# xl-tang3/RCOT

Measured on AMD Instinct MI355X. Metric: 128x128 patches/sec (gen+critic step), higher is better.
Workload: dtype fp32 (exact fp32 MFMA everywhere); 1 GPU; BASELINE configs[1]: Restormer T_net(decoder=True)+F_net(128), denoise_50, RMSprop, paired, B=8/GPU 128x128; global_batch=8, patch=128, parallelism=dp1, gemm_prec=fp32

## Files before the change

### rcot_amd/csrc/pointwise.hip

```cpp
#include <cstdlib>
#include "common.h"
#include "../../include/rcot_hip.h"

using namespace rcot;

namespace {

constexpr int LN_TX = 16, LN_TY = 16, LN_PIX = LN_TX * 4;

__device__ __forceinline__ float4 f4_add(float4 a, float4 b) { return make_float4(a.x + b.x, a.y + b.y, a.z + b.z, a.w + b.w); }

template <int TX>
__device__ __forceinline__ float4 reduce_rows(float4 v, float4* red, int tx, int ty) {
    constexpr int TY = 256 / TX;
    __syncthreads();
    red[ty * TX + tx] = v;
    __syncthreads();
    float4 t = red[tx];
#pragma unroll
    for (int i = 1; i < TY; ++i) t = f4_add(t, red[i * TX + tx]);
    return t;
}

__global__ __launch_bounds__(256) void ln_stats_kernel(const float* __restrict__ x, float* __restrict__ mu,
                                                       float* __restrict__ rs, int C, int N) {
    __shared__ float4 red[256];
    const int tx = threadIdx.x & (LN_TX - 1), ty = threadIdx.x >> 4;
    const int n = blockIdx.x * LN_PIX + tx * 4;
    const int b = blockIdx.y;
    const bool ok = n < N;
    const float* p = x + (long)b * C * N + (ok ? n : 0);
    const float4 sh = ok ? *reinterpret_cast<const float4*>(p) : make_float4(0, 0, 0, 0);
    float4 s = make_float4(0, 0, 0, 0), ss = make_float4(0, 0, 0, 0);
    if (ok) {
#pragma unroll 4
        for (int c = ty; c < C; c += LN_TY) {
            const float4 v = *reinterpret_cast<const float4*>(p + (long)c * N);
            const float dx_ = v.x - sh.x, dy_ = v.y - sh.y, dz_ = v.z - sh.z, dw_ = v.w - sh.w;
            s.x += dx_; s.y += dy_; s.z += dz_; s.w += dw_;
            ss.x += dx_ * dx_; ss.y += dy_ * dy_; ss.z += dz_ * dz_; ss.w += dw_ * dw_;
        }
    }
    s = reduce_rows<LN_TX>(s, red, tx, ty);
    ss = reduce_rows<LN_TX>(ss, red, tx, ty);
    if (ty == 0 && ok) {
        const float inv = 1.0f / (float)C;
        float4 m, r;
#define RCOT_LN_FIN(q)                                              \
    {                                                               \
        const float e = s.q * inv;                                  \
        const float var = fmaxf(ss.q * inv - e * e, 0.f);           \
        m.q = sh.q + e;                                             \
        r.q = 1.0f / sqrtf(var + 1e-5f);                            \
    }
        RCOT_LN_FIN(x) RCOT_LN_FIN(y) RCOT_LN_FIN(z) RCOT_LN_FIN(w)
#undef RCOT_LN_FIN
        *reinterpret_cast<float4*>(mu + (long)b * N + n) = m;
        *reinterpret_cast<float4*>(rs + (long)b * N + n) = r;
    }
}

template <int NC, int TX>
__global__ __launch_bounds__(256) void ln_bwd_kernel(const float* __restrict__ g, const float* __restrict__ x,
                                                     const float* __restrict__ mu, const float* __restrict__ rs,
                                                     const float* __restrict__ w, const float* __restrict__ dres,
                                                     float* __restrict__ dx, float* __restrict__ part, int C, int N) {
    constexpr int TY = 256 / TX, PIX = TX * 4;
    __shared__ float4 red[256];
    __shared__ float sdw[512], sdb[512];
    const int tid = threadIdx.x;
    const int tx = tid % TX, ty = tid / TX;
    const int b = blockIdx.y;
    for (int c = tid; c < C; c += 256) { sdw[c] = 0.f; sdb[c] = 0.f; }
    __syncthreads();
    const int ntiles = (N + PIX - 1) / PIX;
    for (int tile = blockIdx.x; tile < ntiles; tile += gridDim.x) {
        const int n = tile * PIX + tx * 4;
        const bool ok = n < N;
        const long base = (long)b * C * N + (ok ? n : 0);
        const float4 m = ok ? *reinterpret_cast<const float4*>(mu + (long)b * N + n) : make_float4(0, 0, 0, 0);
        const float4 r = ok ? *reinterpret_cast<const float4*>(rs + (long)b * N + n) : make_float4(0, 0, 0, 0);
        float4 s1 = make_float4(0, 0, 0, 0), s2 = make_float4(0, 0, 0, 0);
        constexpr int NR = NC > 0 ? NC : 1;
        float4 gk[NR], xk[NR];
        const int niter = NC > 0 ? NC : (C - ty + TY - 1) / TY;
#pragma unroll
        for (int it = 0; it < NR; ++it) { gk[it] = make_float4(0, 0, 0, 0); xk[it] = gk[it]; }
        if (NC > 0 && ok) {
#pragma unroll
            for (int it = 0; it < NR; ++it) {
                const long i = base + (long)(ty + it * TY) * N;
                gk[it] = *reinterpret_cast<const float4*>(g + i);
                xk[it] = *reinterpret_cast<const float4*>(x + i);
            }
        }
        for (int it = 0; it < niter; ++it) {
            const int c = ty + it * TY;
            float4 gv = make_float4(0, 0, 0, 0), xh = gv;
            if (NC > 0) {
#pragma unroll
                for (int q = 0; q < NR; ++q)
                    if (q == it) { gv = gk[q]; xh = xk[q]; }
                xh = make_float4((xh.x - m.x) * r.x, (xh.y - m.y) * r.y, (xh.z - m.z) * r.z, (xh.w - m.w) * r.w);
#pragma unroll
                for (int q = 0; q < NR; ++q)
                    if (q == it) xk[q] = xh;
            } else if (ok) {
                gv = *reinterpret_cast<const float4*>(g + base + (long)c * N);
                const float4 xv = *reinterpret_cast<const float4*>(x + base + (long)c * N);
                xh = make_float4((xv.x - m.x) * r.x, (xv.y - m.y) * r.y, (xv.z - m.z) * r.z, (xv.w - m.w) * r.w);
            }
            const float wc = w[c];
            s1.x += gv.x * wc; s1.y += gv.y * wc; s1.z += gv.z * wc; s1.w += gv.w * wc;
            s2.x += gv.x * wc * xh.x; s2.y += gv.y * wc * xh.y; s2.z += gv.z * wc * xh.z; s2.w += gv.w * wc * xh.w;
            float a = gv.x * xh.x + gv.y * xh.y + gv.z * xh.z + gv.w * xh.w;
            float bb = gv.x + gv.y + gv.z + gv.w;
#pragma unroll
            for (int o = TX / 2; o > 0; o >>= 1) {
                a += __shfl_xor(a, o, 64);
                bb += __shfl_xor(bb, o, 64);
            }
            if (tx == 0) {
                sdw[c] += a;
                sdb[c] += bb;
            }
        }
        s1 = reduce_rows<TX>(s1, red, tx, ty);
        s2 = reduce_rows<TX>(s2, red, tx, ty);
        if (ok) {
            const float inv = 1.0f / (float)C;
            s1.x *= inv; s1.y *= inv; s1.z *= inv; s1.w *= inv;
            s2.x *= inv; s2.y *= inv; s2.z *= inv; s2.w *= inv;
#pragma unroll
            for (int it = 0; it < NR; ++it) {
                if (NC == 0) break;
                const int c = ty + it * TY;
                const long i = base + (long)c * N;
                const float wc = w[c];
                float4 v;
                v.x = r.x * (gk[it].x * wc - s1.x - xk[it].x * s2.x);
                v.y = r.y * (gk[it].y * wc - s1.y - xk[it].y * s2.y);
                v.z = r.z * (gk[it].z * wc - s1.z - xk[it].z * s2.z);
                v.w = r.w * (gk[it].w * wc - s1.w - xk[it].w * s2.w);
                if (dres) v = f4_add(v, *reinterpret_cast<const float4*>(dres + i));
                *reinterpret_cast<float4*>(dx + i) = v;
            }
            if (NC == 0)
                for (int c = ty; c < C; c += TY) {
                    const long i = base + (long)c * N;
                    const float4 gv = *reinterpret_cast<const float4*>(g + i);
                    const float4 xv = *reinterpret_cast<const float4*>(x + i);
                    const float wc = w[c];
                    float4 v;
                    v.x = r.x * (gv.x * wc - s1.x - (xv.x - m.x) * r.x * s2.x);
                    v.y = r.y * (gv.y * wc - s1.y - (xv.y - m.y) * r.y * s2.y);
                    v.z = r.z * (gv.z * wc - s1.z - (xv.z - m.z) * r.z * s2.z);
                    v.w = r.w * (gv.w * wc - s1.w - (xv.w - m.w) * r.w * s2.w);
                    if (dres) v = f4_add(v, *reinterpret_cast<const float4*>(dres + i));
                    *reinterpret_cast<float4*>(dx + i) = v;
                }
        }
    }
    __syncthreads();
    float* row = part + ((long)blockIdx.y * gridDim.x + blockIdx.x) * (2 * C);
    for (int c = tid; c < C; c += 256) {
        row[c] = sdw[c];
        row[C + c] = sdb[c];
    }
}

__global__ __launch_bounds__(1024) void ln_param_reduce_kernel(const float* __restrict__ part, int rows, int C,
                                                               float* __restrict__ dw, float* __restrict__ db) {
    __shared__ float red[32][33];
    const int cl = threadIdx.x & 31, rl = threadIdx.x >> 5;
    const int col = blockIdx.x * 32 + cl, C2 = 2 * C;
    float s0 = 0.f, s1 = 0.f;
    if (col < C2) {
        const float* p = part + col;
        int r = rl;
        for (; r + 32 < rows; r += 64) {
            s0 += p[(long)r * C2];
            s1 += p[(long)(r + 32) * C2];
        }
        if (r < rows) s0 += p[(long)r * C2];
    }
    red[rl][cl] = s0 + s1;
    __syncthreads();
    if (rl == 0 && col < C2) {
        float s = 0.f;
#pragma unroll
        for (int i = 0; i < 32; ++i) s += red[i][cl];
        if (col < C) dw[col] += s;
        else db[col - C] += s;
    }
}

struct SlabSets {
    const float* ws[4];
    float* dst[4];
    int S[4], M[4], N[4], ldws[4];
    int per[4];
    long ldd[4];
    int chunk0[5];
    int n;
};

__global__ __launch_bounds__(1024) void block_param_reduce_kernel(const float* __restrict__ part1, const float* __restrict__ part2,
                                                                  int rows, int C, float* __restrict__ gw1, float* __restrict__ gb1,
                                                                  float* __restrict__ gw2, float* __restrict__ gb2,
                                                                  const float* __restrict__ dWo_part, float* __restrict__ gWo,
                                                                  const float* __restrict__ dtemp_part, float* __restrict__ gtemp,
                                                                  int B, int heads, int nw, SlabSets ss) {
    __shared__ float red[32][33];
    const int nl = (2 * C + 31) / 32;
    const int blk = blockIdx.x;
    if (blk >= 2 * nl + nw) {
        const int cb = blk - 2 * nl - nw;
        int d = 0;
        while (d + 1 < ss.n && cb >= ss.chunk0[d + 1]) ++d;
        const int c = cb - ss.chunk0[d];
        const long mn = (long)ss.M[d] * ss.N[d];
        const long slab = (long)ss.M[d] * ss.ldws[d];
        if (ss.S[d] <= 8) {
            const unsigned Nn = (unsigned)ss.N[d], mnu = (unsigned)mn, S = (unsigned)ss.S[d];
            const unsigned ldw = (unsigned)ss.ldws[d];
            const float* wsb = ss.ws[d];
            float* dstb = ss.dst[d];
            float v[4][8], old[4];
            long doff[4];
            bool ok[4];
#pragma unroll
            for (int j = 0; j < 4; ++j) {
                const unsigned idx = (unsigned)c * 4096u + 1024u * j + threadIdx.x;
                ok[j] = idx < mnu;
                const unsigned ic = ok[j] ? idx : mnu - 1;
                const unsigned m = ic / Nn, n = ic - m * Nn;
                const float* w = wsb + (size_t)m * ldw + n;
                doff[j] = (long)m * ss.ldd[d] + n;
#pragma unroll
                for (unsigned u = 0; u < 8; ++u) {
                    const unsigned uc = u < S ? u : S - 1;
                    v[j][u] = w[(long)uc * slab];
                }
                old[j] = dstb[doff[j]];
            }
#pragma unroll
            for (int j = 0; j < 4; ++j) {
#pragma unroll
                for (unsigned u = 0; u < 8; ++u) v[j][u] = u < S ? v[j][u] : 0.f;
                const float sum = ((v[j][0] + v[j][1]) + (v[j][2] + v[j][3])) + ((v[j][4] + v[j][5]) + (v[j][6] + v[j][7]));
                if (ok[j]) dstb[doff[j]] = old[j] + sum;
            }
            return;
        }
        if (ss.per[d] == 256) {
            const int o = threadIdx.x & 255, q = threadIdx.x >> 8;
            const long idx = (long)c * 256 + o;
            float* part = &red[0][0];
            float a = 0.f;
            int m = 0, n = 0;
            if (idx < mn) {
                m = (int)(idx / ss.N[d]);
                n = (int)(idx - (long)m * ss.N[d]);
                const float* w = ss.ws[d] + (long)m * ss.ldws[d] + n;
                float acc8[8];
#pragma unroll
                for (int u = 0; u < 8; ++u) acc8[u] = 0.f;
                int s = q;
                for (; s + 28 < ss.S[d]; s += 32) {
#pragma unroll
                    for (int u = 0; u < 8; ++u) acc8[u] += w[(long)(s + 4 * u) * slab];
                }
                for (; s < ss.S[d]; s += 4) acc8[0] += w[(long)s * slab];
                a = ((acc8[0] + acc8[1]) + (acc8[2] + acc8[3])) + ((acc8[4] + acc8[5]) + (acc8[6] + acc8[7]));
            }
            part[q * 256 + o] = a;
            __syncthreads();
            if (q == 0 && idx < mn)
                ss.dst[d][(long)m * ss.ldd[d] + n] += (part[o] + part[256 + o]) + (part[512 + o] + part[768 + o]);
            return;
        }
        const int o = threadIdx.x & 255, q = threadIdx.x >> 8;
        const unsigned Nn = (unsigned)ss.N[d], mnu = (unsigned)mn, ldw = (unsigned)ss.ldws[d];
        const int S = ss.S[d];
        float a[4];
        long doff[4];
        bool ok[4];
        const float* w[4];
#pragma unroll
        for (int j = 0; j < 4; ++j) {
            const unsigned idx = (unsigned)c * 1024u + 256u * j + o;
            ok[j] = idx < mnu;
            const unsigned ic = ok[j] ? idx : mnu - 1;
            const unsigned m = ic / Nn, n = ic - m * Nn;
            w[j] = ss.ws[d] + (size_t)m * ldw + n;
            doff[j] = (long)m * ss.ldd[d] + n;
        }
        float acc8[4][8];
#pragma unroll
        for (int j = 0; j < 4; ++j)
#pragma unroll
            for (int u = 0; u < 8; ++u) acc8[j][u] = 0.f;
        int sl = q;
        for (; sl + 28 < S; sl += 32) {
#pragma unroll
            for (int j = 0; j < 4; ++j)
#pragma unroll
                for (int u = 0; u < 8; ++u) acc8[j][u] += w[j][(long)(sl + 4 * u) * slab];
        }
        for (; sl < S; sl += 4) {
#pragma unroll
            for (int j = 0; j < 4; ++j) acc8[j][0] += w[j][(long)sl * slab];
        }
#pragma unroll
        for (int j = 0; j < 4; ++j)
            a[j] = ((acc8[j][0] + acc8[j][1]) + (acc8[j][2] + acc8[j][3])) + ((acc8[j][4] + acc8[j][5]) + (acc8[j][6] + acc8[j][7]));
        __shared__ float part4[4][1024];
#pragma unroll
        for (int j = 0; j < 4; ++j) part4[q][256 * j + o] = a[j];
        __syncthreads();
        {
            const int t = threadIdx.x;
            const unsigned idx = (unsigned)c * 1024u + t;
            if (idx < mnu) {
                const unsigned m = idx / Nn, n = idx - m * Nn;
                ss.dst[d][(long)m * ss.ldd[d] + n] += (part4[0][t] + part4[1][t]) + (part4[2][t] + part4[3][t]);
            }
        }
        (void)doff; (void)ok;
        return;
    }
    if (blk < 2 * nl) {
        const float* part = blk < nl ? part1 : part2;
        float* dw = blk < nl ? gw1 : gw2;
        float* db = blk < nl ? gb1 : gb2;
        const int cb = blk < nl ? blk : blk - nl;
        const int cl = threadIdx.x & 31, rl = threadIdx.x >> 5;
        const int col = cb * 32 + cl, C2 = 2 * C;
        float a8[8];
#pragma unroll
        for (int u = 0; u < 8; ++u) a8[u] = 0.f;
        if (col < C2) {
            const float* p = part + col;
            int r = rl;
            for (; r + 224 < rows; r += 256) {
#pragma unroll
                for (int u = 0; u < 8; ++u) a8[u] += p[(long)(r + 32 * u) * C2];
            }
            for (; r < rows; r += 32) a8[0] += p[(long)r * C2];
        }
        red[rl][cl] = ((a8[0] + a8[1]) + (a8[2] + a8[3])) + ((a8[4] + a8[5]) + (a8[6] + a8[7]));
        __syncthreads();
        if (rl == 0 && col < C2) {
            float s = 0.f;
#pragma unroll
            for (int i = 0; i < 32; ++i) s += red[i][cl];
            if (col < C) dw[col] += s;
            else db[col - C] += s;
        }
        return;
    }
    const long n = (long)C * C;
    const long i = (long)(blk - 2 * nl) * 1024 + threadIdx.x;
    if (i < n) {
        float s = 0.f;
        int b = 0;
        for (; b + 8 <= B; b += 8) {
            float v[8];
#pragma unroll
            for (int u = 0; u < 8; ++u) v[u] = dWo_part[(long)(b + u) * n + i];
#pragma unroll
            for (int u = 0; u < 8; ++u) s += v[u];
        }
        for (; b < B; ++b) s += dWo_part[(long)b * n + i];
        gWo[i] += s;
    }
    if (blk == 2 * nl && threadIdx.x < heads) {
        float s = 0.f;
        for (int b = 0; b < B; ++b) s += dtemp_part[(long)b * heads + threadIdx.x];
        gtemp[threadIdx.x] += s;
    }
}

__global__ __launch_bounds__(256) void row_sumsq_kernel(const float* __restrict__ x, float* __restrict__ out, int R,
                                                        int N, long sXb) {
    __shared__ float red[4];
    const int r = blockIdx.x, b = blockIdx.y;
    const float* p = x + (long)b * sXb + (long)r * N;
    float s = 0.f;
#pragma unroll 4
    for (int n = threadIdx.x * 4; n < N; n += 1024) {
        const float4 v = *reinterpret_cast<const float4*>(p + n);
        s += v.x * v.x + v.y * v.y + v.z * v.z + v.w * v.w;
    }
    s = block_sum<256>(s, red);
    if (threadIdx.x == 0) out[(long)b * R + r] = s;
}

__global__ void lrelu_bwd_kernel(const float* __restrict__ dy, const float* __restrict__ a, float* __restrict__ dz,
                                 long n, float slope) {
    for (long i = (long)blockIdx.x * blockDim.x + threadIdx.x; i < n; i += (long)gridDim.x * blockDim.x)
        dz[i] = a[i] > 0.f ? dy[i] : dy[i] * slope;
}

__global__ __launch_bounds__(256) void bias_grad_kernel(const float* __restrict__ dz, float* __restrict__ db, int B,
                                                        int C, int P) {
    __shared__ float red[4];
    const int c = blockIdx.x;
    float s = 0.f;
    for (int b = 0; b < B; ++b) {
        const float* p = dz + ((long)b * C + c) * P;
#pragma unroll 8
        for (int i = threadIdx.x; i < P; i += 256) s += p[i];
    }
    s = block_sum<256>(s, red);
    if (threadIdx.x == 0) atomicAdd(&db[c], s);
}

__global__ void axpby2d_kernel(const float* x, long sx, const float* y, long sy, float* out, long so, long rows,
                               long cols, float a, float b) {
    const long n = rows * cols;
    for (long i = (long)blockIdx.x * blockDim.x + threadIdx.x; i < n; i += (long)gridDim.x * blockDim.x) {
        const long r = i / cols, c = i - r * cols;
        out[r * so + c] = a * x[r * sx + c] + (y ? b * y[r * sy + c] : 0.f);
    }
}

__global__ void fill_kernel(float* __restrict__ p, long n, float v) {
    const long head = min(n, (long)((4 - (((uintptr_t)p >> 2) & 3)) & 3));
    const long n4 = (n - head) >> 2;
    float4* q = reinterpret_cast<float4*>(p + head);
    const float4 v4 = make_float4(v, v, v, v);
    const long t0 = (long)blockIdx.x * blockDim.x + threadIdx.x, ts = (long)gridDim.x * blockDim.x;
    for (long i = t0; i < n4; i += ts) q[i] = v4;
    if (t0 < head) p[t0] = v;
    const long tail = head + 4 * n4;
    if (t0 < n - tail) p[tail + t0] = v;
}

__global__ void lerp_kernel(const float* __restrict__ t, const float* __restrict__ f, const float* __restrict__ alpha,
                            float* __restrict__ out, long per, long n) {
    for (long i = (long)blockIdx.x * blockDim.x + threadIdx.x; i < n; i += (long)gridDim.x * blockDim.x) {
        const float a = alpha[i / per];
        out[i] = a * t[i] + (1.f - a) * f[i];
    }
}

__global__ __launch_bounds__(256) void gp_norm_kernel(const float* __restrict__ g, float* __restrict__ norms, long per) {
    __shared__ float red[4];
    const float* p = g + (long)blockIdx.x * per;
    float s = 0.f;
    for (long i = threadIdx.x; i < per; i += 256) s += p[i] * p[i];
    s = block_sum<256>(s, red);
    if (threadIdx.x == 0) norms[blockIdx.x] = sqrtf(s);
}
__global__ void gp_scale_kernel(const float* __restrict__ g, const float* __restrict__ norms, float* __restrict__ u0,
                                float* __restrict__ gp_out, long per, int B, float inv_bg) {
    const long n = per * B;
    if (blockIdx.x == 0 && threadIdx.x == 0) {
        float s = 0.f;
        for (int b = 0; b < B; ++b) s += (norms[b] - 1.f) * (norms[b] - 1.f);
        *gp_out = 10.f * inv_bg * s;
    }
    for (long i = (long)blockIdx.x * blockDim.x + threadIdx.x; i < n; i += (long)gridDim.x * blockDim.x) {
        const float nm = norms[i / per];
        const float coef = nm > 0.f ? 20.f * inv_bg * (nm - 1.f) / nm : 0.f;
        u0[i] = coef * g[i];
    }
}

__global__ void pixel_shuffle_kernel(const float* __restrict__ in, float* __restrict__ out, long n, int H, int W, int mode) {
    for (long i = (long)blockIdx.x * blockDim.x + threadIdx.x; i < n; i += (long)gridDim.x * blockDim.x) {
        const int x = (int)(i % W);
        const long t = i / W;
        const int y = (int)(t % H);
        const long ch = t / H;
        long o;
        if (mode == 1) {
            const long oc = 4 * ch + 2 * (y & 1) + (x & 1);
            o = (oc * (H >> 1) + (y >> 1)) * (W >> 1) + (x >> 1);
        } else {
            const long oc = ch >> 2;
            const int ii = (int)((ch >> 1) & 1), jj = (int)(ch & 1);
            o = (oc * (2 * H) + (2 * y + ii)) * (2L * W) + (2 * x + jj);
        }
        out[o] = in[i];
    }
}

inline int ln_bwd_grid(int B, int N, bool* wide) {
    *wide = (long)cdiv(N, 64) * B >= 512;
    const int tiles = cdiv(N, *wide ? 64 : 16);
    int gx = 1024 / B;
    if (gx < 1) gx = 1;
    if (gx > tiles) gx = tiles;
    return gx;
}

}

extern "C" {

int rcot_ln_stats(const float* x, float* mu, float* rs, int B, int C, int N, void* stream) {
    if (!x || !mu || !rs || B <= 0 || C <= 0 || N <= 0) return RCOT_EINVAL;
    if ((N & 3) || (reinterpret_cast<uintptr_t>(x) & 15) || (reinterpret_cast<uintptr_t>(mu) & 15) ||
        (reinterpret_cast<uintptr_t>(rs) & 15))
        return RCOT_EINVAL;
    RCOT_LAUNCH(ln_stats_kernel, dim3(cdiv(N, LN_PIX), B), dim3(256), 0, (hipStream_t)stream, x, mu, rs, C, N);
    RCOT_LAUNCH_CHECK();
    return RCOT_OK;
}

int rcot_ln_bwd(const float* g, const float* x, const float* mu, const float* rs, const float* w, const float* dres,
                float* dx, float* dw, float* db, int B, int C, int N, void* ws, long ws_bytes, void* stream) {
    if (!g || !x || !mu || !rs || !w || !dx || !ws || B <= 0 || C <= 0 || C > 512 || N <= 0 || B > 65535) return RCOT_EINVAL;
    if ((dw == nullptr) != (db == nullptr)) return RCOT_EINVAL;
    if ((N & 3) || !al16(g) || !al16(x) || !al16(mu) || !al16(rs) || !al16(dx) || !al16(dres)) return RCOT_EINVAL;
    bool wide;
    const int gx = ln_bwd_grid(B, N, &wide);
    const long need = (long)gx * B * 2 * C * (long)sizeof(float);
    if (ws_bytes < need) return RCOT_EINVAL;
    float* part = static_cast<float*>(ws);
    const dim3 grid(gx, B);
    const int TY = wide ? 16 : 64;
    const int nc = (C % TY == 0 && (C / TY == 3 || C / TY == 6)) ? C / TY : 0;
#define RCOT_LNB(NC, TX) do { note_kernel("ln_bwd_kernel<%d, %d>", NC, TX); RCOT_LAUNCH((ln_bwd_kernel<NC, TX>), grid, dim3(256), 0, (hipStream_t)stream, g, x, mu, rs, w, dres, dx, part, C, N); } while (0)
    if (wide) {
        if (nc == 3) RCOT_LNB(3, 16);
        else if (nc == 6) RCOT_LNB(6, 16);
        else RCOT_LNB(0, 16);
    } else {
        if (nc == 3) RCOT_LNB(3, 4);
        else if (nc == 6) RCOT_LNB(6, 4);
        else RCOT_LNB(0, 4);
    }
#undef RCOT_LNB
    RCOT_LAUNCH_CHECK();
    if (dw) {
        RCOT_LAUNCH(ln_param_reduce_kernel, dim3(cdiv(2 * C, 32)), dim3(1024), 0, (hipStream_t)stream, part, gx * B, C, dw, db);
        RCOT_LAUNCH_CHECK();
    }
    return RCOT_OK;
}

int rcot_ln_bwd_rows(int B, int C, int N) {
    (void)C;
    if (B <= 0 || N <= 0) return 0;
    bool wide;
    return ln_bwd_grid(B, N, &wide) * B;
}

int rcot_block_param_reduce(const float* part1, const float* part2, int rows, int C, float* gw1, float* gb1, float* gw2,
                            float* gb2, const float* dWo_part, float* gWo, const float* dtemp_part, float* gtemp, int B,
                            int heads, const long long* slab_sets, int n_sets, void* stream) {
    if (!part1 || !part2 || !gw1 || !gb1 || !gw2 || !gb2 || !dWo_part || !gWo || !dtemp_part || !gtemp || rows <= 0 || C <= 0 ||
        B <= 0 || heads <= 0 || heads > 1024 || n_sets < 0 || n_sets > 4 || (n_sets && !slab_sets))
        return RCOT_EINVAL;
    const int nl = cdiv(2 * C, 32);
    const int nw = cdiv((long)C * C, 1024);
    SlabSets ss{};
    ss.n = n_sets;
    int chunks = 0;
    for (int d = 0; d < n_sets; ++d) {
        const long long* r = slab_sets + 7 * d;
        ss.ws[d] = reinterpret_cast<const float*>(r[0]);
        ss.S[d] = (int)r[1]; ss.M[d] = (int)r[2]; ss.N[d] = (int)r[3]; ss.ldws[d] = (int)r[4];
        ss.dst[d] = reinterpret_cast<float*>(r[5]);
        ss.ldd[d] = r[6];
        if (!ss.ws[d] || !ss.dst[d] || ss.S[d] <= 0 || ss.M[d] <= 0 || ss.N[d] <= 0 || ss.ldws[d] < ss.N[d]) return RCOT_EINVAL;
        ss.chunk0[d] = chunks;
        const long mn_ = (long)ss.M[d] * ss.N[d];
        ss.per[d] = ss.S[d] <= 8 ? 4096 : (mn_ >= 256 * 1024 ? 1024 : 256);
        chunks += cdiv(mn_, ss.per[d]);
    }
    ss.chunk0[n_sets] = chunks;
    RCOT_LAUNCH(block_param_reduce_kernel, dim3(2 * nl + nw + chunks), dim3(1024), 0, (hipStream_t)stream, part1, part2, rows,
                       C, gw1, gb1, gw2, gb2, dWo_part, gWo, dtemp_part, gtemp, B, heads, nw, ss);
    RCOT_LAUNCH_CHECK();
    return RCOT_OK;
}

int rcot_row_sumsq(const float* x, float* out, int B, int R, int N, long sXb, void* stream) {
    if (!x || !out || B <= 0 || R <= 0 || N <= 0 || (N & 3) || (sXb & 3) || !al16(x) || B > 65535) return RCOT_EINVAL;
    RCOT_LAUNCH(row_sumsq_kernel, dim3(R, B), dim3(256), 0, (hipStream_t)stream, x, out, R, N, sXb);
    RCOT_LAUNCH_CHECK();
    return RCOT_OK;
}

int rcot_lrelu_bwd(const float* dy, const float* a, float* dz, long n, float slope, void* stream) {
    if (!dy || !a || !dz || n <= 0) return RCOT_EINVAL;
    RCOT_LAUNCH(lrelu_bwd_kernel, dim3(grid_for(n)), dim3(256), 0, (hipStream_t)stream, dy, a, dz, n, slope);
    RCOT_LAUNCH_CHECK();
    return RCOT_OK;
}

int rcot_bias_grad(const float* dz, float* db, int B, int C, int P, void* stream) {
    if (!dz || !db || B <= 0 || C <= 0 || P <= 0) return RCOT_EINVAL;
    RCOT_LAUNCH(bias_grad_kernel, dim3(C), dim3(256), 0, (hipStream_t)stream, dz, db, B, C, P);
    RCOT_LAUNCH_CHECK();
    return RCOT_OK;
}

int rcot_axpby2d(const float* x, long sx, const float* y, long sy, float* out, long so, long rows, long cols, float a,
                 float b, void* stream) {
    if (!x || !out || rows <= 0 || cols <= 0) return RCOT_EINVAL;
    RCOT_LAUNCH(axpby2d_kernel, dim3(grid_for(rows * cols)), dim3(256), 0, (hipStream_t)stream, x, sx, y, sy, out,
                       so, rows, cols, a, b);
    RCOT_LAUNCH_CHECK();
    return RCOT_OK;
}

int rcot_fill(float* p, long n, float v, void* stream) {
    if (!p || n <= 0) return RCOT_EINVAL;
    RCOT_LAUNCH(fill_kernel, dim3(grid_for((n + 3) / 4)), dim3(256), 0, (hipStream_t)stream, p, n, v);
    RCOT_LAUNCH_CHECK();
    return RCOT_OK;
}

int rcot_lerp(const float* t, const float* f, const float* alpha, float* out, int B, long per, void* stream) {
    if (!t || !f || !alpha || !out || B <= 0 || per <= 0) return RCOT_EINVAL;
    RCOT_LAUNCH(lerp_kernel, dim3(grid_for(per * B)), dim3(256), 0, (hipStream_t)stream, t, f, alpha, out, per, per * B);
    RCOT_LAUNCH_CHECK();
    return RCOT_OK;
}

int rcot_gp_penalty(const float* g, float* norms, float* u0, float* gp_out, int B, long per, float inv_global_batch,
                    void* stream) {
    if (!g || !norms || !u0 || !gp_out || B <= 0 || per <= 0) return RCOT_EINVAL;
    RCOT_LAUNCH(gp_norm_kernel, dim3(B), dim3(256), 0, (hipStream_t)stream, g, norms, per);
    RCOT_LAUNCH_CHECK();
    RCOT_LAUNCH(gp_scale_kernel, dim3(grid_for(per * B)), dim3(256), 0, (hipStream_t)stream, g, norms, u0, gp_out,
                       per, B, inv_global_batch);
    RCOT_LAUNCH_CHECK();
    return RCOT_OK;
}

int rcot_pixel_shuffle(const float* in, float* out, long planes, int H, int W, int mode, void* stream) {
    if (!in || !out || planes <= 0 || H <= 0 || W <= 0 || (mode != 1 && mode != 2)) return RCOT_EINVAL;
    if (mode == 1 && ((H | W) & 1)) return RCOT_EINVAL;
    if (mode == 2 && (planes & 3)) return RCOT_EINVAL;
    const long n = planes * H * W;
    RCOT_LAUNCH(pixel_shuffle_kernel, dim3(grid_for(n)), dim3(256), 0, (hipStream_t)stream, in, out, n, H, W, mode);
    RCOT_LAUNCH_CHECK();
    return RCOT_OK;
}

}
```

Baseline: 107.2 patches/s.

## Restructure LayerNorm backward with register-held channels, wider blocks, and warp-shuffle reductions

Rewrites the LayerNorm backward kernel so the per-channel weight/bias gradient partials stay in registers across tiles instead of shared-memory accumulators. Block size now scales with C (256/512/1024 threads) so each thread holds a fixed 3 channels, with the residual gradient also loaded into registers. The column reductions for s1/s2 now use cross-lane shuffles plus a double-buffered small shared array with one barrier per tile. The kernel also uses 32-bit byte offsets and a waves-per-EU hint. This is meant to cut LDS traffic, barriers and reloads of g/x. In exchange there are more template variants and more register pressure.

```diff
diff --git a/rcot_amd/csrc/pointwise.hip b/rcot_amd/csrc/pointwise.hip
--- a/rcot_amd/csrc/pointwise.hip
+++ b/rcot_amd/csrc/pointwise.hip
@@ -60,112 +60,172 @@
     }
 }
 
-template <int NC, int TX>
-__global__ __launch_bounds__(256) void ln_bwd_kernel(const float* __restrict__ g, const float* __restrict__ x,
-                                                     const float* __restrict__ mu, const float* __restrict__ rs,
-                                                     const float* __restrict__ w, const float* __restrict__ dres,
-                                                     float* __restrict__ dx, float* __restrict__ part, int C, int N) {
-    constexpr int TY = 256 / TX, PIX = TX * 4;
-    __shared__ float4 red[256];
-    __shared__ float sdw[512], sdb[512];
+template <int LO, int HI>
+__device__ __forceinline__ float4 lanes_sum(float4 v) {
+#pragma unroll
+    for (int o = LO; o < HI; o <<= 1)
+        v = make_float4(v.x + __shfl_xor(v.x, o, 64), v.y + __shfl_xor(v.y, o, 64), v.z + __shfl_xor(v.z, o, 64),
+                        v.w + __shfl_xor(v.w, o, 64));
+    return v;
+}
+
+__device__ __forceinline__ float4 ldf4(const float* p) { return *reinterpret_cast<const float4*>(p); }
+__device__ __forceinline__ float4 ldf4(const float* base, unsigned byte_off) {
+    return *reinterpret_cast<const float4*>(reinterpret_cast<const char*>(base) + byte_off);
+}
+
+template <int NC, int TX, int NT, bool REG, bool DR>
+__global__ __launch_bounds__(NT) __attribute__((amdgpu_waves_per_eu(REG && NT < 1024 ? 5 : 4)))
+void ln_bwd_kernel(const float* __restrict__ g, const float* __restrict__ x, const float* __restrict__ mu,
+                   const float* __restrict__ rs, const float* __restrict__ w, const float* __restrict__ dres,
+                   float* __restrict__ dx, float* __restrict__ part, int C, int N) {
+    constexpr int TY = NT / TX, PIX = TX * 4, NW = NT / 64;
+    constexpr int G = 64 / TX < NW ? 64 / TX : NW;
+    constexpr int CH = TY >= 64 ? 2 : 4;
+    static_assert(REG || NC % CH == 0, "whole chunks");
+    __shared__ float4 red[2][NW][2][TX];
     const int tid = threadIdx.x;
-    const int tx = tid % TX, ty = tid / TX;
+    const int tx = tid % TX, ty = tid / TX, wv = tid / 64;
+    const int rw = (tid & 63) / TX;
+    const bool lead = rw == 0;
     const int b = blockIdx.y;
-    for (int c = tid; c < C; c += 256) { sdw[c] = 0.f; sdb[c] = 0.f; }
-    __syncthreads();
+    const float inv = 1.0f / (float)C;
+    g += (long)b * C * N;
+    x += (long)b * C * N;
+    if (DR) dres += (long)b * C * N;
+    dx += (long)b * C * N;
+    mu += (long)b * N;
+    rs += (long)b * N;
+    float aw[NC], ab[NC], wk[NC];
+    unsigned co[REG ? NC : 1];
+#pragma unroll
+    for (int it = 0; it < NC; ++it) {
+        const int c = ty + it * TY;
+        aw[it] = 0.f;
+        ab[it] = 0.f;
+        wk[it] = c < C ? w[c < C ? c : 0] : 0.f;
+        if (REG) co[it] = (unsigned)c * (unsigned)N * 4u;
+    }
     const int ntiles = (N + PIX - 1) / PIX;
-    for (int tile = blockIdx.x; tile < ntiles; tile += gridDim.x) {
+    int par = 0;
+    for (int tile = blockIdx.x; tile < ntiles; tile += gridDim.x, par ^= 1) {
         const int n = tile * PIX + tx * 4;
         const bool ok = n < N;
-        const long base = (long)b * C * N + (ok ? n : 0);
-        const float4 m = ok ? *reinterpret_cast<const float4*>(mu + (long)b * N + n) : make_float4(0, 0, 0, 0);
-        const float4 r = ok ? *reinterpret_cast<const float4*>(rs + (long)b * N + n) : make_float4(0, 0, 0, 0);
-        float4 s1 = make_float4(0, 0, 0, 0), s2 = make_float4(0, 0, 0, 0);
-        constexpr int NR = NC > 0 ? NC : 1;
-        float4 gk[NR], xk[NR];
-        const int niter = NC > 0 ? NC : (C - ty + TY - 1) / TY;
-#pragma unroll
-        for (int it = 0; it < NR; ++it) { gk[it] = make_float4(0, 0, 0, 0); xk[it] = gk[it]; }
-        if (NC > 0 && ok) {
+        const int nc = ok ? n : 0;
+        constexpr int NR = REG ? NC : 1;
+        float4 gk[NR], xk[NR], dk[NR];
+        if (REG) {
 #pragma unroll
             for (int it = 0; it < NR; ++it) {
-                const long i = base + (long)(ty + it * TY) * N;
-                gk[it] = *reinterpret_cast<const float4*>(g + i);
-                xk[it] = *reinterpret_cast<const float4*>(x + i);
-            }
-        }
-        for (int it = 0; it < niter; ++it) {
-            const int c = ty + it * TY;
-            float4 gv = make_float4(0, 0, 0, 0), xh = gv;
-            if (NC > 0) {
-#pragma unroll
-                for (int q = 0; q < NR; ++q)
-                    if (q == it) { gv = gk[q]; xh = xk[q]; }
-                xh = make_float4((xh.x - m.x) * r.x, (xh.y - m.y) * r.y, (xh.z - m.z) * r.z, (xh.w - m.w) * r.w);
-#pragma unroll
-                for (int q = 0; q < NR; ++q)
-                    if (q == it) xk[q] = xh;
-            } else if (ok) {
-                gv = *reinterpret_cast<const float4*>(g + base + (long)c * N);
-                const float4 xv = *reinterpret_cast<const float4*>(x + base + (long)c * N);
-                xh = make_float4((xv.x - m.x) * r.x, (xv.y - m.y) * r.y, (xv.z - m.z) * r.z, (xv.w - m.w) * r.w);
-            }
-            const float wc = w[c];
-            s1.x += gv.x * wc; s1.y += gv.y * wc; s1.z += gv.z * wc; s1.w += gv.w * wc;
-            s2.x += gv.x * wc * xh.x; s2.y += gv.y * wc * xh.y; s2.z += gv.z * wc * xh.z; s2.w += gv.w * wc * xh.w;
-            float a = gv.x * xh.x + gv.y * xh.y + gv.z * xh.z + gv.w * xh.w;
-            float bb = gv.x + gv.y + gv.z + gv.w;
-#pragma unroll
-            for (int o = TX / 2; o > 0; o >>= 1) {
-                a += __shfl_xor(a, o, 64);
-                bb += __shfl_xor(bb, o, 64);
-            }
-            if (tx == 0) {
-                sdw[c] += a;
-                sdb[c] += bb;
-            }
-        }
-        s1 = reduce_rows<TX>(s1, red, tx, ty);
-        s2 = reduce_rows<TX>(s2, red, tx, ty);
-        if (ok) {
-            const float inv = 1.0f / (float)C;
-            s1.x *= inv; s1.y *= inv; s1.z *= inv; s1.w *= inv;
-            s2.x *= inv; s2.y *= inv; s2.z *= inv; s2.w *= inv;
+                const unsigned i = co[it] + 4u * nc;
+                gk[it] = ldf4(g, i);
+                xk[it] = ldf4(x, i);
+                if (DR) dk[it] = ldf4(dres, i);
+            }
+        }
+        const float4 m = ldf4(mu + nc), r = ldf4(rs + nc);
+        float4 s1 = make_float4(0, 0, 0, 0), s2 = s1;
+#define RCOT_LNB_ACC(it, gv, xv, gw, xh)                                                                                    \
+    {                                                                                                                       \
+        xh = make_float4((xv.x - m.x) * r.x, (xv.y - m.y) * r.y, (xv.z - m.z) * r.z, (xv.w - m.w) * r.w);                   \
+        const float a = gv.x * xh.x + gv.y * xh.y + gv.z * xh.z + gv.w * xh.w;                                              \
+        const float bb = gv.x + gv.y + gv.z + gv.w;                                                                         \
+        aw[it] += ok ? a : 0.f;                                                                                             \
+        ab[it] += ok ? bb : 0.f;                                                                                            \
+        gw = make_float4(gv.x * wk[it], gv.y * wk[it], gv.z * wk[it], gv.w * wk[it]);                                       \
+        s1.x += gw.x; s1.y += gw.y; s1.z += gw.z; s1.w += gw.w;                                                             \
+        s2.x += gw.x * xh.x; s2.y += gw.y * xh.y; s2.z += gw.z * xh.z; s2.w += gw.w * xh.w;                                 \
+    }
+        if (REG) {
 #pragma unroll
             for (int it = 0; it < NR; ++it) {
-                if (NC == 0) break;
-                const int c = ty + it * TY;
-                const long i = base + (long)c * N;
+                const float4 gv = gk[it], xv = xk[it];
+                RCOT_LNB_ACC(it, gv, xv, gk[it], xk[it])
+            }
+#pragma unroll
+            for (int it = 0; it < NR; ++it) asm volatile("" : "+v"(aw[it]), "+v"(ab[it]));
+        } else {
+#pragma unroll
+            for (int i0 = 0; i0 < NC; i0 += CH) {
+                if (i0 * TY >= C) break;
+                float4 gc[CH], xc[CH];
+#pragma unroll
+                for (int q = 0; q < CH; ++q) {
+                    const int c = ty + (i0 + q) * TY;
+                    const long i = (long)(c < C ? c : C - 1) * N + nc;
+                    gc[q] = ldf4(g + i);
+                    xc[q] = ldf4(x + i);
+                }
+#pragma unroll
+                for (int q = 0; q < CH; ++q) {
+                    float4 gw, xh;
+                    RCOT_LNB_ACC(i0 + q, gc[q], xc[q], gw, xh)
+                }
+            }
+        }
+#undef RCOT_LNB_ACC
+        s1 = lanes_sum<TX, 64>(s1);
+        s2 = lanes_sum<TX, 64>(s2);
+        if (lead) {
+            red[par][wv][0][tx] = s1;
+            red[par][wv][1][tx] = s2;
+        }
+        __syncthreads();
+        s1 = red[par][rw % G][0][tx];
+        s2 = red[par][rw % G][1][tx];
+#pragma unroll
+        for (int q = G; q < NW; q += G) {
+            s1 = f4_add(s1, red[par][rw % G + q][0][tx]);
+            s2 = f4_add(s2, red[par][rw % G + q][1][tx]);
+        }
+        s1 = lanes_sum<TX, TX * G>(s1);
+        s2 = lanes_sum<TX, TX * G>(s2);
+        s1.x *= inv; s1.y *= inv; s1.z *= inv; s1.w *= inv;
+        s2.x *= inv; s2.y *= inv; s2.z *= inv; s2.w *= inv;
+        if (REG) {
+#pragma unroll
+            for (int it = 0; it < NR; ++it) {
+                float4 v;
+                v.x = r.x * (gk[it].x - s1.x - xk[it].x * s2.x);
+                v.y = r.y * (gk[it].y - s1.y - xk[it].y * s2.y);
+                v.z = r.z * (gk[it].z - s1.z - xk[it].z * s2.z);
+                v.w = r.w * (gk[it].w - s1.w - xk[it].w * s2.w);
+                if (DR) v = f4_add(v, dk[it]);
+                if (ok) *reinterpret_cast<float4*>(reinterpret_cast<char*>(dx) + (co[it] + 4u * nc)) = v;
+            }
+        } else {
+#pragma unroll 2
+            for (int c = ty; c < C; c += TY) {
+                const long i = (long)c * N + nc;
+                const float4 gv = ldf4(g + i), xv = ldf4(x + i);
                 const float wc = w[c];
                 float4 v;
-                v.x = r.x * (gk[it].x * wc - s1.x - xk[it].x * s2.x);
-                v.y = r.y * (gk[it].y * wc - s1.y - xk[it].y * s2.y);
-                v.z = r.z * (gk[it].z * wc - s1.z - xk[it].z * s2.z);
-                v.w = r.w * (gk[it].w * wc - s1.w - xk[it].w * s2.w);
-                if (dres) v = f4_add(v, *reinterpret_cast<const float4*>(dres + i));
-                *reinterpret_cast<float4*>(dx + i) = v;
-            }
-            if (NC == 0)
-                for (int c = ty; c < C; c += TY) {
-                    const long i = base + (long)c * N;
-                    const float4 gv = *reinterpret_cast<const float4*>(g + i);
-                    const float4 xv = *reinterpret_cast<const float4*>(x + i);
-                    const float wc = w[c];
-                    float4 v;
-                    v.x = r.x * (gv.x * wc - s1.x - (xv.x - m.x) * r.x * s2.x);
-                    v.y = r.y * (gv.y * wc - s1.y - (xv.y - m.y) * r.y * s2.y);
-                    v.z = r.z * (gv.z * wc - s1.z - (xv.z - m.z) * r.z * s2.z);
-                    v.w = r.w * (gv.w * wc - s1.w - (xv.w - m.w) * r.w * s2.w);
-                    if (dres) v = f4_add(v, *reinterpret_cast<const float4*>(dres + i));
-                    *reinterpret_cast<float4*>(dx + i) = v;
-                }
-        }
-    }
-    __syncthreads();
-    float* row = part + ((long)blockIdx.y * gridDim.x + blockIdx.x) * (2 * C);
-    for (int c = tid; c < C; c += 256) {
-        row[c] = sdw[c];
-        row[C + c] = sdb[c];
+                v.x = r.x * (gv.x * wc - s1.x - (xv.x - m.x) * r.x * s2.x);
+                v.y = r.y * (gv.y * wc - s1.y - (xv.y - m.y) * r.y * s2.y);
+                v.z = r.z * (gv.z * wc - s1.z - (xv.z - m.z) * r.z * s2.z);
+                v.w = r.w * (gv.w * wc - s1.w - (xv.w - m.w) * r.w * s2.w);
+                if (DR) v = f4_add(v, ldf4(dres + i));
+                if (ok) *reinterpret_cast<float4*>(dx + i) = v;
+            }
+        }
+    }
+#pragma unroll
+    for (int it = 0; it < NC; ++it)
+#pragma unroll
+        for (int o = TX / 2; o > 0; o >>= 1) {
+            aw[it] += __shfl_xor(aw[it], o, 64);
+            ab[it] += __shfl_xor(ab[it], o, 64);
+        }
+    if (tx == 0) {
+        float* row = part + ((long)blockIdx.y * gridDim.x + blockIdx.x) * (2 * C);
+#pragma unroll
+        for (int it = 0; it < NC; ++it) {
+            const int c = ty + it * TY;
+            if (c < C) {
+                row[c] = aw[it];
+                row[C + c] = ab[it];
+            }
+        }
     }
 }
 
@@ -488,13 +548,28 @@
     }
 }
 
-inline int ln_bwd_grid(int B, int N, bool* wide) {
-    *wide = (long)cdiv(N, 64) * B >= 512;
-    const int tiles = cdiv(N, *wide ? 64 : 16);
-    int gx = 1024 / B;
-    if (gx < 1) gx = 1;
-    if (gx > tiles) gx = tiles;
-    return gx;
+constexpr int LN_BWD_ROWS = 1024;
+struct LnBwdForm { int nc, tx, nt; bool reg; int gx; };
+inline LnBwdForm ln_bwd_form(int B, int C, int N) {
+    LnBwdForm f;
+    const bool off32 = (long)C * N < (1L << 30);
+    if ((long)cdiv(N, 64) * B >= 512) {
+        if (!off32) f = {8, 16, 1024, false, 0};
+        else if (C == 48) f = {3, 16, 256, true, 0};
+        else if (C == 96) f = {3, 16, 512, true, 0};
+        else if (C == 192) f = {3, 16, 1024, true, 0};
+        else f = {8, 16, 1024, false, 0};
+    } else {
+        if (!off32) f = {8, 4, 256, false, 0};
+        else if (C == 192) f = {3, 4, 256, true, 0};
+        else if (C == 384) f = {3, 4, 512, true, 0};
+        else f = {8, 4, 256, false, 0};
+    }
+    const int tiles = cdiv(N, 4 * f.tx);
+    f.gx = LN_BWD_ROWS / B;
+    if (f.gx < 1) f.gx = 1;
+    if (f.gx > tiles) f.gx = tiles;
+    return f;
 }
 
 }
@@ -516,25 +591,26 @@
     if (!g || !x || !mu || !rs || !w || !dx || !ws || B <= 0 || C <= 0 || C > 512 || N <= 0 || B > 65535) return RCOT_EINVAL;
     if ((dw == nullptr) != (db == nullptr)) return RCOT_EINVAL;
     if ((N & 3) || !al16(g) || !al16(x) || !al16(mu) || !al16(rs) || !al16(dx) || !al16(dres)) return RCOT_EINVAL;
-    bool wide;
-    const int gx = ln_bwd_grid(B, N, &wide);
+    const LnBwdForm f = ln_bwd_form(B, C, N);
+    const int gx = f.gx;
     const long need = (long)gx * B * 2 * C * (long)sizeof(float);
     if (ws_bytes < need) return RCOT_EINVAL;
     float* part = static_cast<float*>(ws);
     const dim3 grid(gx, B);
-    const int TY = wide ? 16 : 64;
-    const int nc = (C % TY == 0 && (C / TY == 3 || C / TY == 6)) ? C / TY : 0;
-#define RCOT_LNB(NC, TX) do { note_kernel("ln_bwd_kernel<%d, %d>", NC, TX); RCOT_LAUNCH((ln_bwd_kernel<NC, TX>), grid, dim3(256), 0, (hipStream_t)stream, g, x, mu, rs, w, dres, dx, part, C, N); } while (0)
-    if (wide) {
-        if (nc == 3) RCOT_LNB(3, 16);
-        else if (nc == 6) RCOT_LNB(6, 16);
-        else RCOT_LNB(0, 16);
+#define RCOT_LNB2(NC, TX, NT, REG, DR) do { note_kernel("ln_bwd_kernel<%d, %d, %d, %s, %s>", NC, TX, NT, #REG, #DR); RCOT_LAUNCH((ln_bwd_kernel<NC, TX, NT, REG, DR>), grid, dim3(NT), 0, (hipStream_t)stream, g, x, mu, rs, w, dres, dx, part, C, N); } while (0)
+#define RCOT_LNB(NC, TX, NT, REG) do { if (dres) RCOT_LNB2(NC, TX, NT, REG, true); else RCOT_LNB2(NC, TX, NT, REG, false); } while (0)
+    if (f.tx == 16) {
+        if (!f.reg) RCOT_LNB(8, 16, 1024, false);
+        else if (f.nt == 256) RCOT_LNB(3, 16, 256, true);
+        else if (f.nt == 512) RCOT_LNB(3, 16, 512, true);
+        else RCOT_LNB(3, 16, 1024, true);
     } else {
-        if (nc == 3) RCOT_LNB(3, 4);
-        else if (nc == 6) RCOT_LNB(6, 4);
-        else RCOT_LNB(0, 4);
+        if (!f.reg) RCOT_LNB(8, 4, 256, false);
+        else if (f.nt == 256) RCOT_LNB(3, 4, 256, true);
+        else RCOT_LNB(3, 4, 512, true);
     }
 #undef RCOT_LNB
+#undef RCOT_LNB2
     RCOT_LAUNCH_CHECK();
     if (dw) {
         RCOT_LAUNCH(ln_param_reduce_kernel, dim3(cdiv(2 * C, 32)), dim3(1024), 0, (hipStream_t)stream, part, gx * B, C, dw, db);
@@ -544,10 +620,8 @@
 }
 
 int rcot_ln_bwd_rows(int B, int C, int N) {
-    (void)C;
     if (B <= 0 || N <= 0) return 0;
-    bool wide;
-    return ln_bwd_grid(B, N, &wide) * B;
+    return ln_bwd_form(B, C, N).gx * B;
 }
 
 int rcot_block_param_reduce(const float* part1, const float* part2, int rows, int C, float* gw1, float* gb1, float* gw2,
```

Result: no change. 107.7 patches/s (median of 6 runs) (+0.5%).
